# kotaro-kinoshita/yomitoku

Measured on AMD Instinct MI355X. Metric: pages/sec (DocumentAnalyzer @1600x1200, lite model set), higher is better.
Workload: dtype f32 held as two scaled fp16 planes per operand on the MFMA pipe: 3 x v_mfma_f32_32x32x16_f16 per product tile (products to 2^-21, below the fp32 accumulation's own rounding), fp32 accumulate, fp32 activations in HBM; attention, LayerNorm, the fused greedy step and every grid-starved launch exact fp3

## Files before the change

yomitoku_amd/csrc/ymk_api.cpp:

```cpp
#include "../../include/ymk.h"
#include "ymk_common.h"
#include "ymk_decstep.h"
#include "ymk_det.h"
#include "ymk_entry.h"
#include "ymk_seq.h"

struct ymk_model {
  ymk::Model* impl = nullptr;
  int device = 0;
};

#include <dlfcn.h>
namespace {
struct Roctx {
  int (*push)(const char*) = nullptr;
  int (*pop)() = nullptr;
  Roctx() {
    const char* on = std::getenv("YMK_ROCTX");
    if (on == nullptr || on[0] == '\0' || on[0] == '0') return;
    for (const char* name : {"librocprofiler-sdk-roctx.so", "libroctx64.so"}) {
      if (void* h = dlopen(name, RTLD_NOW | RTLD_GLOBAL)) {
        push = reinterpret_cast<int (*)(const char*)>(dlsym(h, "roctxRangePushA"));
        pop = reinterpret_cast<int (*)()>(dlsym(h, "roctxRangePop"));
        if (push && pop) return;
// ... 26 lines not shown
    return 1;                                       \
  }                                                 \
  catch (...) {                                     \
    ymk::set_error("unknown C++ exception");        \
    return 2;                                       \
  }

extern "C" {

int ymk_version(void) { return 100; }

const char* ymk_last_error(void) { return ymk::last_error().c_str(); }

int ymk_device_count(void) {
  int n = 0;
  if (hipGetDeviceCount(&n) != hipSuccess) return -1;
  return n;
}

ymk_model* ymk_model_create(const char* kind, int device) {
  try {
    YMK_CHECK(kind != nullptr, "kind is null");
    YMK_HIP(hipSetDevice(device));
    std::string k(kind);
    ymk::Model* impl = nullptr;
    if (k == "dbnet") impl = ymk::create_dbnet();
    else if (k == "parseq") impl = ymk::create_parseq();
    else if (k == "rtdetr") impl = ymk::create_rtdetr();
    else throw ymk::Error("unknown model kind: " + k);
    auto* m = new ymk_model();
    m->impl = impl;
    m->device = device;
    return m;
  } catch (const std::exception& e) {
    ymk::set_error(e.what());
    return nullptr;
  }
}

void ymk_model_destroy(ymk_model* m) {
  if (!m) return;
  (void)hipSetDevice(m->device);
  delete m->impl;
  delete m;
}

int ymk_model_set_param(ymk_model* m, const char* key, double value) {
  YMK_API_BEGIN
  YMK_CHECK(m && key, "null argument");
  const std::string k(key);
  if (k == "workspace_reuse") {
    YMK_CHECK(value == 0.0 || value == 1.0 || value == -1.0, "workspace_reuse must be 0 or 1 (-1: follow the process-wide default)");
    YMK_CHECK(!ymk::in_forward(), "workspace_reuse cannot change inside a forward");
  }
  m->impl->params[key] = value;
  if (m->impl->finalized && (k == "conv_split" || k == "conv_split_encoder")) {
    YMK_HIP(hipSetDevice(m->device));
    m->impl->prebuild_split();
  }
  YMK_API_END
}

int ymk_model_set_tensor(ymk_model* m, const char* name, const float* host_data, int ndim, const int64_t* dims) {
  YMK_API_BEGIN
  YMK_CHECK(m && name && host_data && (ndim == 0 || dims), "null argument");
  YMK_CHECK(!m->impl->finalized, "model already finalized");
  m->impl->ws.put(name, host_data, ndim, dims);
  YMK_API_END
}

int ymk_model_finalize(ymk_model* m) {
  YMK_API_BEGIN
  RoctxRange roctx_range("ymk_model_finalize");
  YMK_CHECK(m, "null model");
  YMK_HIP(hipSetDevice(m->device));
  m->impl->finalize();
  m->impl->prebuild_split();
  if (!ymk::debug_hazard_no_finalize_sync()) YMK_HIP(hipDeviceSynchronize());
  YMK_API_END
}

int ymk_model_reserve(ymk_model* m, int n, int h, int w, void* stream) {
  YMK_API_BEGIN
  RoctxRange roctx_range("ymk_model_reserve");
  YMK_CHECK(m && m->impl, "null argument");
  YMK_HIP(hipSetDevice(m->device));
  m->impl->reserve(n, h, w, (hipStream_t)stream);
  YMK_API_END
}

int64_t ymk_model_weight_bytes(const ymk_model* m) { return m ? (int64_t)m->impl->pool.bytes() : -1; }
int64_t ymk_model_workspace_bytes(const ymk_model* m) { return m ? (int64_t)m->impl->arena.capacity() : -1; }

int ymk_dbnet_forward(ymk_model* m, const float* x_dev, int n, int h, int w, float* prob_dev, void* stream) {
  YMK_API_BEGIN
  RoctxRange roctx_range("ymk_dbnet_forward");
  YMK_CHECK(m && x_dev && prob_dev, "null argument");
  YMK_HIP(hipSetDevice(m->device));
  ymk::dbnet_forward(m->impl, x_dev, n, h, w, prob_dev, (hipStream_t)stream);
  YMK_API_END
}

int ymk_parseq_dims(ymk_model* m, int* num_steps, int* num_classes) {
  YMK_API_BEGIN
  YMK_CHECK(m && num_steps && num_classes, "null argument");
  ymk::parseq_dims(m->impl, num_steps, num_classes);
  YMK_API_END
}

int ymk_parseq_forward(ymk_model* m, const float* x_dev, int b, int w, float* logits_dev, int* out_len, int* ar_steps,
                       void* stream) {
  YMK_API_BEGIN
  RoctxRange roctx_range("ymk_parseq_forward");
  YMK_CHECK(m && x_dev && logits_dev && out_len && ar_steps, "null argument");
  YMK_HIP(hipSetDevice(m->device));
  ymk::parseq_forward(m->impl, x_dev, b, w, logits_dev, out_len, ar_steps, (hipStream_t)stream);
  YMK_API_END
}

int ymk_parseq_forward_groups(ymk_model* m, const float* const* x_dev, const int* b, const int* w, int n_groups,
                              float* logits_dev, int* out_len, int* ar_steps, void* stream) {
  YMK_API_BEGIN
  RoctxRange roctx_range("ymk_parseq_forward_groups");
  YMK_CHECK(m && x_dev && b && w && logits_dev && out_len && ar_steps, "null argument");
  YMK_HIP(hipSetDevice(m->device));
  ymk::parseq_forward_groups(m->impl, x_dev, b, w, n_groups, logits_dev, out_len, ar_steps, (hipStream_t)stream);
  YMK_API_END
}

int ymk_parseq_token_stats(const float* logits_dev, int rows, int num_classes, int* ids_dev, float* probs_dev,
                           void* stream) {
  YMK_API_BEGIN
  RoctxRange roctx_range("ymk_parseq_token_stats");
  YMK_CHECK(logits_dev && ids_dev && probs_dev, "null argument");
  ymk::row_maxprob((hipStream_t)stream, logits_dev, rows, num_classes, ids_dev, probs_dev);
  YMK_API_END
}

int ymk_rtdetr_forward(ymk_model* m, const float* x_dev, int b, int h, int w, float* logits_dev, float* boxes_dev,
                       void* stream) {
  YMK_API_BEGIN
  RoctxRange roctx_range("ymk_rtdetr_forward");
  YMK_CHECK(m && x_dev && logits_dev && boxes_dev, "null argument");
  YMK_HIP(hipSetDevice(m->device));
  ymk::rtdetr_forward(m->impl, x_dev, b, h, w, logits_dev, boxes_dev, (hipStream_t)stream);
  YMK_API_END
}

int ymk_debug_option(const char* key, int value) {
  YMK_API_BEGIN
  YMK_CHECK(key != nullptr, "null key");
  const std::string k(key);
  YMK_CHECK(ymk::conv_debug_option(k, value) || ymk::parseq_debug_option(k, value) || ymk::decstep_debug_option(k, value) ||
                ymk::conv_split_debug_option(k, value) || ymk::runtime_debug_option(k, value),
            "unknown debug option: " + k);
  YMK_API_END
}

int ymk_stat(const char* key, int64_t* value) {
  YMK_API_BEGIN
  YMK_CHECK(key != nullptr && value != nullptr, "null argument");
  long long v = 0;
  YMK_CHECK(ymk::conv_split_stat(std::string(key), &v) || ymk::runtime_stat(std::string(key), &v) || ymk::parseq_stat(std::string(key), &v), std::string("unknown counter: ") + key);
  *value = v;
  YMK_API_END
}

int ymk_amax_check_counters(int64_t* out4) {
  YMK_API_BEGIN
  YMK_CHECK(out4 != nullptr, "null argument");
  long long v[4];
  ymk::amax_check_counters(v);
  for (int i = 0; i < 4; ++i) out4[i] = v[i];
  YMK_API_END
}

int ymk_prof_begin(void) {
  YMK_API_BEGIN
  ymk::prof_begin();
  YMK_API_END
}

int ymk_prof_end(double* conv_ms, double* conv_flop, int64_t* conv_launches) {
  YMK_API_BEGIN
  YMK_CHECK(conv_ms && conv_flop && conv_launches, "null argument");
  ymk::prof_end(conv_ms, conv_flop, conv_launches);
  YMK_API_END
}

int ymk_prof_bytes(double* conv_bytes) {
  YMK_API_BEGIN
  YMK_CHECK(conv_bytes, "null argument");
  *conv_bytes = ymk::prof_bytes();
  YMK_API_END
}

int ymk_prof_launch_table(double* ms, double* flop, double* bytes, double* mfma_products, int64_t capacity, int64_t* count) {
  YMK_API_BEGIN
  YMK_CHECK(count != nullptr && capacity >= 0 && (capacity == 0 || (ms && flop && bytes && mfma_products)), "null argument");
  *count = ymk::prof_launch_table(ms, flop, bytes, mfma_products, capacity);
  YMK_API_END
}

int ymk_op_plan_workspace(int64_t n, const int64_t* sizes, const int64_t* release_pos, int64_t* offsets_out, int64_t* peak_out,
                          int64_t* live_bound_out) {
  YMK_API_BEGIN
  YMK_CHECK(n >= 0 && (n == 0 || (sizes && offsets_out)), "plan_workspace: bad argument");
  std::vector<size_t> sz((size_t)n), off((size_t)n);
  for (int64_t k = 0; k < n; ++k) {
    YMK_CHECK(sizes[k] >= 0, "plan_workspace: negative size");
    sz[(size_t)k] = (size_t)sizes[k];
  }
  size_t peak = 0, live = 0;
  ymk::plan_workspace((size_t)n, sz.data(), release_pos, off.data(), &peak, &live);
  for (int64_t k = 0; k < n; ++k) offsets_out[k] = (int64_t)off[(size_t)k];
  if (peak_out) *peak_out = (int64_t)peak;
  if (live_bound_out) *live_bound_out = (int64_t)live;
  YMK_API_END
}

int ymk_op_conv2d(const float* x_dev, int n, int h, int w, int c, const float* w_host_oihw, int cout, int cin, int kh,
                  int kw, const float* scale_host, const float* bias_host, const float* res_dev, int stride, int pad,
                  int dil, int act, int tap4, float* y_dev, void* stream) {
  YMK_API_BEGIN
  using namespace ymk;
  DevicePool pool;
  ConvW cw;
  cw.cout = cout;
  cw.cin = tap4 ? 4 : cin;
  cw.kh = kh;
  cw.kw = kw;
  cw.mode = tap4 ? 1 : 0;
  std::vector<float> panel;
  pack_conv_weight(w_host_oihw, cout, cin, kh, kw, tap4 != 0, panel, cw.kpad, cw.ctiles);
  cw.w = pool.upload(panel);
  if (scale_host) cw.scale = pool.upload(scale_host, cout);
  if (bias_host) cw.bias = pool.upload(bias_host, cout);
  Tensor in{const_cast<float*>(x_dev), n, h, w, c, c};
  const int oh = conv_out_dim(h, kh, stride, pad, dil), ow = conv_out_dim(w, kw, stride, pad, dil);
  Tensor out{y_dev, n, oh, ow, cout, cout};
  Tensor res{const_cast<float*>(res_dev), n, oh, ow, cout, cout};
  ConvArgs a;
  a.stride = stride;
  a.pad = pad;
  a.dil = dil;
  a.act = act;
  a.res = res_dev ? &res : nullptr;
  SplitCtxOwner split_ctx;
  ConvSplitScope scope(-1, split_ctx.get(), 0);
  conv2d((hipStream_t)stream, in, cw, a, out);
  YMK_HIP(hipStreamSynchronize((hipStream_t)stream));
  YMK_API_END
}

int ymk_op_conv1x1_astat(const float* x_dev, int m, int c, const float* w_host_oc, int cout, const float* scale_host,
                         const float* bias_host, const float* res_dev, int act, const float* ln_g_host, const float* ln_b_host, float ln_eps,
                         float* y_dev, int reps, float* kernel_ms, void* stream) {
  YMK_API_BEGIN
  using namespace ymk;
  YMK_CHECK(x_dev && w_host_oc && y_dev && m > 0 && c > 0 && cout > 0, "bad argument");
  YMK_CHECK((ln_g_host == nullptr) == (ln_b_host == nullptr), "LayerNorm: gamma and beta come together");
  hipStream_t s = (hipStream_t)stream;
  DevicePool pool;
  ConvW cw;
  cw.cout = cout;
  cw.cin = c;
  std::vector<float> panel;
  YMK_CHECK(c % 4 == 0, "astat: channels must be a multiple of 4");
  pack_conv_weight(w_host_oc, cout, c, 1, 1, false, panel, cw.kpad, cw.ctiles);
  YMK_CHECK(cw.kpad <= 256, "astat: K <= 256");
  cw.w = pool.upload(panel);
  if (scale_host) cw.scale = pool.upload(scale_host, cout);
  if (bias_host) cw.bias = pool.upload(bias_host, cout);
  unsigned* rec = nullptr;
  const float *g_dev = nullptr, *b_dev = nullptr;
  if (ln_g_host) {
    const std::vector<float> g(ln_g_host, ln_g_host + c), b(ln_b_host, ln_b_host + c);
    g_dev = pool.upload(g);
    b_dev = pool.upload(b);
    rec = make_layernorm_amax_record(pool, g, b);
  } else {
    rec = reinterpret_cast<unsigned*>(pool.alloc(AMAX_REC_WORDS));
    YMK_HIP(hipMemsetAsync(rec, 0, AMAX_REC_WORDS * sizeof(unsigned), s));
    absmax_record(s, x_dev, (size_t)m * c, rec);
  }
  struct Events {
    hipEvent_t e0 = nullptr, e1 = nullptr;
    ~Events() {
      if (e0) (void)hipEventDestroy(e0);
      if (e1) (void)hipEventDestroy(e1);
    }
  } ev;
  YMK_HIP(hipEventCreate(&ev.e0));
  YMK_HIP(hipEventCreate(&ev.e1));
  SplitCtxOwner split_ctx;
  ConvSplitScope scope(SPLIT_F16X2, split_ctx.get(), 0);
  ConvSplitTileScope tile_scope(30);
  for (int r = 0; r < std::max(1, reps); ++r) {
    if (r == std::max(1, reps) - 1) YMK_HIP(hipEventRecord(ev.e0, s));
    if (ln_g_host) {
      YMK_CHECK(gemm_ln_fused(s, x_dev, m, c, c, g_dev, b_dev, ln_eps, cw, act, res_dev, cout, y_dev, cout, rec),
                "astat: this launch cannot carry a fused LayerNorm (C must be 128 or 192)");
    } else {
      YMK_CHECK(gemm_takes_astat(m, c, cw, res_dev != nullptr, cout), "astat: not a launch the A-stationary kernel runs");
      gemm(s, x_dev, m, c, c, cw, act, res_dev, cout, y_dev, cout, nullptr, nullptr, EPI_STORE, rec);
    }
    if (r == std::max(1, reps) - 1) YMK_HIP(hipEventRecord(ev.e1, s));
  }
  YMK_HIP(hipStreamSynchronize(s));
  float ms = 0.f;
  YMK_HIP(hipEventElapsedTime(&ms, ev.e0, ev.e1));
  if (kernel_ms) *kernel_ms = ms;
  YMK_API_END
}

int ymk_op_vit_mlp(const float* x_dev, int m, int d, int f, const float* ln_g_host, const float* ln_b_host, float ln_eps,
// ... 365 lines not shown
```

yomitoku_amd/csrc/ymk_entry.h:

```cpp
#pragma once
#include "ymk_common.h"

namespace ymk {

void dbnet_forward(Model* m, const float* x, int n, int h, int w, float* prob, hipStream_t s);
Model* create_parseq();
void parseq_forward(Model* m, const float* x, int B, int W, float* logits, int* out_len, int* ar_steps, hipStream_t s);
void parseq_forward_groups(Model* m, const float* const* x, const int* b, const int* w, int ng, float* logits, int* out_len,
                           int* ar_steps, hipStream_t s);
void parseq_dims(Model* m, int* num_steps, int* num_classes);
bool parseq_debug_option(const std::string& key, int value);
bool parseq_stat(const std::string& key, long long* value);
Model* create_rtdetr();
void rtdetr_forward(Model* m, const float* x, int B, int H, int W, float* logits, float* boxes, hipStream_t s);

void prof_begin();
void prof_end(double* ms, double* flop, int64_t* launches);
double prof_bytes();
int64_t prof_launch_table(double* ms, double* flop, double* bytes, double* products, int64_t capacity);
bool conv_debug_option(const std::string& key, int value);

bool conv_split_debug_option(const std::string& key, int value);
bool conv_split_stat(const std::string& key, long long* value);
void amax_check_counters(long long* out4);
bool gemm_takes_astat(int M, int K, const ConvW& w, bool with_res, int ld);

}
```

yomitoku_amd/csrc/ymk_seq.hip:

```cpp
#include "ymk_common.h"
#include "ymk_f16_planes.h"
#include "ymk_seq.h"

namespace ymk {


__device__ __forceinline__ float wave_sum(float v) {
#pragma unroll
  for (int o = 32; o > 0; o >>= 1) v += __shfl_xor(v, o, 64);
  return v;
}
__device__ __forceinline__ float wave_max(float v) {
#pragma unroll
  for (int o = 32; o > 0; o >>= 1) v = fmaxf(v, __shfl_xor(v, o, 64));
  return v;
}

__global__ void k_layernorm(const float* __restrict__ x, int ldx, int in_rows_mod, const float* __restrict__ g,
                            const float* __restrict__ b, float eps, float* __restrict__ y, int ldy, int M, int D) {
  const int row = blockIdx.x * (blockDim.x >> 6) + (threadIdx.x >> 6);
  const int lane = threadIdx.x & 63;
  if (row >= M) return;
  const float* xr = x + (size_t)(in_rows_mod > 0 ? row % in_rows_mod : row) * ldx;
  float4 v[4];
  const int nv = D >> 2;
  float s = 0.f;
#pragma unroll
  for (int i = 0; i < 4; ++i) {
    const int c = lane + 64 * i;
    if (c < nv) {
      v[i] = *reinterpret_cast<const float4*>(xr + c * 4);
      s += (v[i].x + v[i].y) + (v[i].z + v[i].w);
    }
  }
  const float mean = wave_sum(s) / (float)D;
  float q = 0.f;
#pragma unroll
  for (int i = 0; i < 4; ++i) {
    const int c = lane + 64 * i;
    if (c < nv) {
      const float a = v[i].x - mean, bb = v[i].y - mean, cc = v[i].z - mean, d = v[i].w - mean;
      q += (a * a + bb * bb) + (cc * cc + d * d);
    }
  }
  const float rstd = 1.f / sqrtf(wave_sum(q) / (float)D + eps);
#pragma unroll
  for (int i = 0; i < 4; ++i) {
    const int c = lane + 64 * i;
    if (c < nv) {
      const float4 gg = *reinterpret_cast<const float4*>(g + c * 4);
      const float4 be = *reinterpret_cast<const float4*>(b + c * 4);
      float4 o;
      o.x = (v[i].x - mean) * rstd * gg.x + be.x;
      o.y = (v[i].y - mean) * rstd * gg.y + be.y;
      o.z = (v[i].z - mean) * rstd * gg.z + be.z;
      o.w = (v[i].w - mean) * rstd * gg.w + be.w;
      *reinterpret_cast<float4*>(y + (size_t)row * ldy + c * 4) = o;
    }
  }
}
void layernorm(hipStream_t s, const float* x, int ldx, int in_rows_mod, const float* g, const float* b, float eps,
               float* y, int ldy, int M, int D) {
  YMK_CHECK(D % 4 == 0 && D <= 1024, "layernorm: D must be a multiple of 4, <= 1024");
  if (M == 0) return;
  hipLaunchKernelGGL(k_layernorm, dim3((M + 3) / 4), dim3(256), 0, s, x, ldx, in_rows_mod, g, b, eps, y, ldy, M, D);
  YMK_HIP(hipGetLastError());
}

__global__ void k_add_pos(float* __restrict__ x, const float* __restrict__ pos, int gh, int gw, int full_gw, int D4,
                          size_t total) {
  for (size_t i = (size_t)blockIdx.x * blockDim.x + threadIdx.x; i < total; i += (size_t)gridDim.x * blockDim.x) {
    const int c4 = (int)(i % D4);
    const size_t tok = i / D4;
    const int cc = (int)(tok % gw);
    const int rr = (int)((tok / gw) % gh);
    float4 v = reinterpret_cast<float4*>(x)[i];
    const float4 p = reinterpret_cast<const float4*>(pos)[(size_t)(rr * full_gw + cc) * D4 + c4];
    v.x += p.x; v.y += p.y; v.z += p.z; v.w += p.w;
    reinterpret_cast<float4*>(x)[i] = v;
  }
}
void add_pos_embed(hipStream_t s, float* x, const float* pos, int B, int gh, int gw, int full_gw, int D) {
  const size_t total = (size_t)B * gh * gw * (D / 4);
  size_t g = (total + 255) / 256;
  if (g > 4096) g = 4096;
  hipLaunchKernelGGL(k_add_pos, dim3((int)g), dim3(256), 0, s, x, pos, gh, gw, full_gw, D / 4, total);
  YMK_HIP(hipGetLastError());
}

struct AttnP {
  const float *q, *k, *v;
  float* o;
  int ldq, ldk, ldv, ldo;
  long bsq, bsk, bsv, bso;
  int Lq, Lk, H;
  float scale;
  const int *qoff, *qlen, *koff, *klen;
  const unsigned *amax_q, *amax_k, *amax_v;
};

template <int HD, int HDR = HD>
__global__ __launch_bounds__(256, 1) void k_flash_attn(AttnP p) {
  constexpr int KT = 64;
  constexpr int LDH = HD + 4;
  constexpr int NKC = HDR / 8;
  constexpr int NDC = HD / 32;
  constexpr int LPT = (KT * HDR / 4) / 256;
  static_assert(HD % 32 == 0 && HDR % 8 == 0 && HDR <= HD && (KT * HDR / 4) % 256 == 0, "head dim");
  __shared__ __attribute__((aligned(16))) float lds[2 * 2 * KT * LDH];

  const int t = threadIdx.x, wv = t >> 6, lane = t & 63, li = lane & 31, lh = lane >> 5;
  const int b = blockIdx.z, h = blockIdx.y;
  const int q0 = blockIdx.x * 128 + wv * 32;
  const float* qb = p.q + (size_t)b * p.bsq + h * HDR;
  const float* kb = p.k + (size_t)b * p.bsk + h * HDR;
  const float* vb = p.v + (size_t)b * p.bsv + h * HDR;
  float* ob = p.o + (size_t)b * p.bso + h * HDR;
  int Lq = p.Lq, Lk = p.Lk;
  if (p.koff) {
    const size_t r = (size_t)p.koff[b];
    kb = p.k + r * p.ldk + h * HDR;
    vb = p.v + r * p.ldv + h * HDR;
    Lk = p.klen[b];
  }
  if (p.qoff) {
    const size_t r = (size_t)p.qoff[b];
    qb = p.q + r * p.ldq + h * HDR;
    ob = p.o + r * p.ldo + h * HDR;
    Lq = p.qlen[b];
  }
  if ((int)blockIdx.x * 128 >= Lq) return;

  f32x4 qf[NKC];
  {
    const int qi = min(q0 + li, Lq - 1);
    const float* qr = qb + (size_t)qi * p.ldq;
#pragma unroll
    for (int kc = 0; kc < NKC; ++kc) {
      qf[kc] = *reinterpret_cast<const f32x4*>(qr + kc * 8 + lh * 4);
      qf[kc] *= p.scale;
    }
  }

  f32x16 oacc[NDC];
#pragma unroll
  for (int dc = 0; dc < NDC; ++dc)
#pragma unroll
    for (int r = 0; r < 16; ++r) oacc[dc][r] = 0.f;
  float m_run = -INFINITY, l_run = 0.f;

  f32x4 rk[LPT], rv[LPT];
  auto load_kv = [&](int k0) {
#pragma unroll
    for (int i = 0; i < LPT; ++i) {
      const int idx = t + 256 * i;
      const int row = idx / (HDR / 4), c4 = idx - row * (HDR / 4);
      const int key = min(k0 + row, Lk - 1);
      rk[i] = *reinterpret_cast<const f32x4*>(kb + (size_t)key * p.ldk + c4 * 4);
      rv[i] = *reinterpret_cast<const f32x4*>(vb + (size_t)key * p.ldv + c4 * 4);
    }
  };
  auto store_kv = [&](int buf) {
    float* Ks = lds + buf * (2 * KT * LDH);
    float* Vs = Ks + KT * LDH;
#pragma unroll
    for (int i = 0; i < LPT; ++i) {
      const int idx = t + 256 * i;
      const int row = idx / (HDR / 4), c4 = idx - row * (HDR / 4);
      *reinterpret_cast<f32x4*>(Ks + row * LDH + c4 * 4) = rk[i];
      *reinterpret_cast<f32x4*>(Vs + row * LDH + c4 * 4) = rv[i];
    }
  };

  const int ntiles = (Lk + KT - 1) / KT;
  load_kv(0);
  store_kv(0);
  __syncthreads();
  for (int tt = 0; tt < ntiles; ++tt) {
    const int buf = tt & 1;
    if (tt + 1 < ntiles) load_kv((tt + 1) * KT);
    const float* Ks = lds + buf * (2 * KT * LDH);
    const float* Vs = Ks + KT * LDH;
#pragma unroll
    for (int sub = 0; sub < (q0 < Lq ? KT / 32 : 0); ++sub) {
      const int kbase = tt * KT + sub * 32;
      if (kbase >= Lk) break;
      f32x16 sacc;
#pragma unroll
      for (int r = 0; r < 16; ++r) sacc[r] = 0.f;
      const float* kr = Ks + (sub * 32 + li) * LDH + lh * 4;
#pragma unroll
      for (int kc = 0; kc < NKC; ++kc) {
        const f32x4 kf = *reinterpret_cast<const f32x4*>(kr + kc * 8);
        sacc = __builtin_amdgcn_mfma_f32_32x32x2f32(kf.x, qf[kc].x, sacc, 0, 0, 0);
        sacc = __builtin_amdgcn_mfma_f32_32x32x2f32(kf.y, qf[kc].y, sacc, 0, 0, 0);
        sacc = __builtin_amdgcn_mfma_f32_32x32x2f32(kf.z, qf[kc].z, sacc, 0, 0, 0);
        sacc = __builtin_amdgcn_mfma_f32_32x32x2f32(kf.w, qf[kc].w, sacc, 0, 0, 0);
      }
      float mt = -INFINITY;
#pragma unroll
      for (int r = 0; r < 16; ++r) {
        const int key = kbase + (r & 3) + 8 * (r >> 2) + 4 * lh;
        if (key >= Lk) sacc[r] = -INFINITY;
        mt = fmaxf(mt, sacc[r]);
      }
      mt = fmaxf(mt, __shfl_xor(mt, 32, 64));
      const float m_new = fmaxf(m_run, mt);
      const float alpha = __expf(m_run - m_new);
      float ps = 0.f;
#pragma unroll
      for (int r = 0; r < 16; ++r) {
        sacc[r] = __expf(sacc[r] - m_new);
        ps += sacc[r];
      }
      ps += __shfl_xor(ps, 32, 64);
      l_run = l_run * alpha + ps;
      m_run = m_new;
#pragma unroll
      for (int dc = 0; dc < NDC; ++dc) {
#pragma unroll
        for (int r = 0; r < 16; ++r) oacc[dc][r] *= alpha;
        const float* vr = Vs + (sub * 32 + 4 * lh) * LDH + dc * 32 + li;
#pragma unroll
        for (int r = 0; r < 16; ++r) {
          const float vf = vr[((r & 3) + 8 * (r >> 2)) * LDH];
          oacc[dc] = __builtin_amdgcn_mfma_f32_32x32x2f32(vf, sacc[r], oacc[dc], 0, 0, 0);
        }
      }
    }
    if (tt + 1 < ntiles) store_kv(buf ^ 1);
    __syncthreads();
  }
  const int qi = q0 + li;
  if (qi < Lq) {
    const float inv = 1.f / l_run;
    float* orow = ob + (size_t)qi * p.ldo;
#pragma unroll
    for (int dc = 0; dc < NDC; ++dc)
#pragma unroll
      for (int g = 0; g < 4; ++g) {
        f32x4 w;
        w.x = oacc[dc][4 * g + 0] * inv;
        w.y = oacc[dc][4 * g + 1] * inv;
        w.z = oacc[dc][4 * g + 2] * inv;
        w.w = oacc[dc][4 * g + 3] * inv;
        if (dc * 32 + 8 * g + 4 * lh < HDR) *reinterpret_cast<f32x4*>(orow + dc * 32 + 8 * g + 4 * lh) = w;
      }
  }
}

template <int HD, int HDR = HD>
__global__ __launch_bounds__(256, (HD <= 32 ? 3 : (HD <= 64 ? 2 : 1))) void k_flash_attn_f16(AttnP p) {
  constexpr int KT = 64;
  constexpr int LDH = HD + 4;
  constexpr int NKS = HDR / 16;
  constexpr int NDC = HD / 32;
  constexpr int LPT = (KT * HDR / 4) / 256;
  static_assert(HD % 32 == 0 && HDR % 16 == 0 && HDR <= HD && (KT * HDR / 4) % 256 == 0, "head dim");
  __shared__ __attribute__((aligned(16))) float lds[2 * 2 * KT * LDH];

  const int t = threadIdx.x, wv = t >> 6, lane = t & 63, li = lane & 31, lh = lane >> 5;
  const int b = blockIdx.z, h = blockIdx.y;
  const int q0 = blockIdx.x * 128 + wv * 32;
  const float* qb = p.q + (size_t)b * p.bsq + h * HDR;
  const float* kb = p.k + (size_t)b * p.bsk + h * HDR;
  const float* vb = p.v + (size_t)b * p.bsv + h * HDR;
  float* ob = p.o + (size_t)b * p.bso + h * HDR;
  int Lq = p.Lq, Lk = p.Lk;
  if (p.koff) {
    const size_t r = (size_t)p.koff[b];
    kb = p.k + r * p.ldk + h * HDR;
    vb = p.v + r * p.ldv + h * HDR;
    Lk = p.klen[b];
  }
  if (p.qoff) {
    const size_t r = (size_t)p.qoff[b];
    qb = p.q + r * p.ldq + h * HDR;
    ob = p.o + r * p.ldo + h * HDR;
    Lq = p.qlen[b];
  }
  if ((int)blockIdx.x * 128 >= Lq) return;

  const float2 cq = f16_plane_scales((unsigned)__builtin_amdgcn_readfirstlane((int)amax_read(p.amax_q, t)));
  const float2 ck = f16_plane_scales((unsigned)__builtin_amdgcn_readfirstlane((int)amax_read(p.amax_k, t)));
  const float2 cv = f16_plane_scales((unsigned)__builtin_amdgcn_readfirstlane((int)amax_read(p.amax_v, t)));
  const float s_q = cq.x, s_k = ck.x, s_v = cv.x;
  const float s_unscale = cq.y * ck.y;
  const float o_unscale = cv.y * (1.f / 16384.f);

  f16x8 qh[NKS], ql[NKS];
  {
    const int qi = min(q0 + li, Lq - 1);
    const float* qr = qb + (size_t)qi * p.ldq;
#pragma unroll
    for (int ks = 0; ks < NKS; ++ks) {
      const f32x4 a = *reinterpret_cast<const f32x4*>(qr + ks * 16 + lh * 8);
      const f32x4 c = *reinterpret_cast<const f32x4*>(qr + ks * 16 + lh * 8 + 4);
      const float x[8] = {a.x * p.scale, a.y * p.scale, a.z * p.scale, a.w * p.scale, c.x * p.scale, c.y * p.scale, c.z * p.scale, c.w * p.scale};
      f16_split8(x, s_q, qh[ks], ql[ks]);
    }
  }

  f32x16 oacc[NDC];
#pragma unroll
  for (int dc = 0; dc < NDC; ++dc)
#pragma unroll
    for (int r = 0; r < 16; ++r) oacc[dc][r] = 0.f;
  float m_run = -INFINITY, l_run = 0.f;

  f32x4 rk[LPT], rv[LPT];
  auto load_kv = [&](int k0) {
#pragma unroll
    for (int i = 0; i < LPT; ++i) {
      const int idx = t + 256 * i;
      const int row = idx / (HDR / 4), c4 = idx - row * (HDR / 4);
      const int key = min(k0 + row, Lk - 1);
      rk[i] = *reinterpret_cast<const f32x4*>(kb + (size_t)key * p.ldk + c4 * 4);
      rv[i] = *reinterpret_cast<const f32x4*>(vb + (size_t)key * p.ldv + c4 * 4);
    }
  };
  auto store_kv = [&](int buf) {
    float* Ks = lds + buf * (2 * KT * LDH);
    float* Vs = Ks + KT * LDH;
#pragma unroll
    for (int i = 0; i < LPT; ++i) {
      const int idx = t + 256 * i;
      const int row = idx / (HDR / 4), c4 = idx - row * (HDR / 4);
      *reinterpret_cast<f32x4*>(Ks + row * LDH + c4 * 4) = rk[i];
      *reinterpret_cast<f32x4*>(Vs + row * LDH + c4 * 4) = rv[i];
    }
  };

  const int ntiles = (Lk + KT - 1) / KT;
  load_kv(0);
  store_kv(0);
  __syncthreads();
  for (int tt = 0; tt < ntiles; ++tt) {
    const int buf = tt & 1;
    if (tt + 1 < ntiles) load_kv((tt + 1) * KT);
    const float* Ks = lds + buf * (2 * KT * LDH);
    const float* Vs = Ks + KT * LDH;
#pragma unroll
    for (int sub = 0; sub < (q0 < Lq ? KT / 32 : 0); ++sub) {
      const int kbase = tt * KT + sub * 32;
      if (kbase >= Lk) break;
      f32x16 sacc;
#pragma unroll
      for (int r = 0; r < 16; ++r) sacc[r] = 0.f;
      const float* kr = Ks + (sub * 32 + li) * LDH + lh * 8;
#pragma unroll
      for (int ks = 0; ks < NKS; ++ks) {
        const f32x4 a = *reinterpret_cast<const f32x4*>(kr + ks * 16);
        const f32x4 c = *reinterpret_cast<const f32x4*>(kr + ks * 16 + 4);
        const float x[8] = {a.x, a.y, a.z, a.w, c.x, c.y, c.z, c.w};
        f16x8 kh, kl;
        f16_split8(x, s_k, kh, kl);
        sacc = __builtin_amdgcn_mfma_f32_32x32x16_f16(kl, qh[ks], sacc, 0, 0, 0);
        sacc = __builtin_amdgcn_mfma_f32_32x32x16_f16(kh, ql[ks], sacc, 0, 0, 0);
        sacc = __builtin_amdgcn_mfma_f32_32x32x16_f16(kh, qh[ks], sacc, 0, 0, 0);
      }
      float mt = -INFINITY;
#pragma unroll
      for (int r = 0; r < 16; ++r) {
        const int key = kbase + (r & 3) + 8 * (r >> 2) + 4 * lh;
        sacc[r] = key >= Lk ? -INFINITY : sacc[r] * s_unscale;
        mt = fmaxf(mt, sacc[r]);
      }
      mt = fmaxf(mt, __shfl_xor(mt, 32, 64));
      const float m_new = fmaxf(m_run, mt);
      const float alpha = __expf(m_run - m_new);
      float ps = 0.f;
#pragma unroll
      for (int r = 0; r < 16; ++r) {
        sacc[r] = __expf(sacc[r] - m_new);
        ps += sacc[r];
      }
      ps += __shfl_xor(ps, 32, 64);
      l_run = l_run * alpha + ps;
      m_run = m_new;
      f16x8 ph[2], pl[2];
#pragma unroll
      for (int j = 0; j < 2; ++j) {
        const float x[8] = {sacc[8 * j], sacc[8 * j + 1], sacc[8 * j + 2], sacc[8 * j + 3], sacc[8 * j + 4], sacc[8 * j + 5], sacc[8 * j + 6], sacc[8 * j + 7]};
        f16_split8(x, 16384.f, ph[j], pl[j]);
      }
#pragma unroll
      for (int dc = 0; dc < NDC; ++dc) {
#pragma unroll
        for (int r = 0; r < 16; ++r) oacc[dc][r] *= alpha;
        const float* vr = Vs + (sub * 32 + 4 * lh) * LDH + dc * 32 + li;
#pragma unroll
        for (int j = 0; j < 2; ++j) {
          float x[8];
#pragma unroll
          for (int e = 0; e < 8; ++e) {
            const int r = 8 * j + e;
            x[e] = vr[((r & 3) + 8 * (r >> 2)) * LDH];
          }
          f16x8 vh, vl;
          f16_split8(x, s_v, vh, vl);
          oacc[dc] = __builtin_amdgcn_mfma_f32_32x32x16_f16(vl, ph[j], oacc[dc], 0, 0, 0);
          oacc[dc] = __builtin_amdgcn_mfma_f32_32x32x16_f16(vh, pl[j], oacc[dc], 0, 0, 0);
          oacc[dc] = __builtin_amdgcn_mfma_f32_32x32x16_f16(vh, ph[j], oacc[dc], 0, 0, 0);
        }
      }
    }
    if (tt + 1 < ntiles) store_kv(buf ^ 1);
    __syncthreads();
  }
  const int qi = q0 + li;
  if (qi < Lq) {
    const float inv = o_unscale / l_run;
    float* orow = ob + (size_t)qi * p.ldo;
#pragma unroll
    for (int dc = 0; dc < NDC; ++dc)
#pragma unroll
      for (int g = 0; g < 4; ++g) {
        f32x4 w;
        w.x = oacc[dc][4 * g + 0] * inv;
        w.y = oacc[dc][4 * g + 1] * inv;
        w.z = oacc[dc][4 * g + 2] * inv;
        w.w = oacc[dc][4 * g + 3] * inv;
        if (dc * 32 + 8 * g + 4 * lh < HDR) *reinterpret_cast<f32x4*>(orow + dc * 32 + 8 * g + 4 * lh) = w;
      }
  }
}

void flash_attention(hipStream_t s, const float* q, const float* k, const float* v, float* o, int B, int H, int Lq, int Lk,
                     int hd, int ldq, int ldk, int ldv, int ldo, long bsq, long bsk, long bsv, long bso, float scale,
                     const SeqTab* tab, const unsigned* amax_q, const unsigned* amax_k, const unsigned* amax_v) {
  if (B == 0 || Lq == 0) return;
  YMK_CHECK(Lk > 0, "attention: no keys");
  YMK_CHECK(ldq % 4 == 0 && ldk % 4 == 0 && ldv % 4 == 0 && ldo % 4 == 0, "attention: strides must be multiples of 4");
  AttnP p{q, k, v, o, ldq, ldk, ldv, ldo, bsq, bsk, bsv, bso, Lq, Lk, H, scale, nullptr, nullptr, nullptr, nullptr, amax_q, amax_k, amax_v};
  if (tab) {
    p.qoff = tab->qoff;
    p.qlen = tab->qlen;
    p.koff = tab->koff;
    p.klen = tab->klen;
    YMK_CHECK((p.qoff == nullptr) == (p.qlen == nullptr) && (p.koff == nullptr) == (p.klen == nullptr), "attention: offset and length tables come in pairs");
  }
  dim3 grid((Lq + 127) / 128, H, B);
  const bool f16 = amax_q && amax_k && amax_v && scale <= 1.f && scale > 0.f && conv_effective_split() == SPLIT_F16X2 && ldq % 4 == 0;
  if (f16 && (hd == 32 || hd == 64 || hd == 96 || hd == 48)) {
    if (hd == 32) hipLaunchKernelGGL(k_flash_attn_f16<32>, grid, dim3(256), 0, s, p);
    else if (hd == 64) hipLaunchKernelGGL(k_flash_attn_f16<64>, grid, dim3(256), 0, s, p);
    else if (hd == 96) hipLaunchKernelGGL(k_flash_attn_f16<96>, grid, dim3(256), 0, s, p);
    else hipLaunchKernelGGL((k_flash_attn_f16<64, 48>), grid, dim3(256), 0, s, p);
    YMK_HIP(hipGetLastError());
    return;
  }
  if (hd == 32) hipLaunchKernelGGL(k_flash_attn<32>, grid, dim3(256), 0, s, p);
  else if (hd == 64) hipLaunchKernelGGL(k_flash_attn<64>, grid, dim3(256), 0, s, p);
  else if (hd == 96) hipLaunchKernelGGL(k_flash_attn<96>, grid, dim3(256), 0, s, p);
  else if (hd == 48) hipLaunchKernelGGL((k_flash_attn<64, 48>), grid, dim3(256), 0, s, p);
  else {
    YMK_CHECK(Lk <= 1024 && hd <= 128, "attention: head dim " + std::to_string(hd) + " is only supported for <= 1024 keys per sample");
    small_attention(s, q, k, v, o, B, H, Lq, Lk, hd, ldq, ldk, ldv, ldo, bsq, bsk, bsv, bso, scale, nullptr, 0, nullptr, 0, tab);
    return;
  }
  YMK_HIP(hipGetLastError());
}

struct SmallAttnP {
  const float *q, *k, *v;
  float* o;
  int ldq, ldk, ldv, ldo;
  long bsq, bsk, bsv, bso;
  int Lq, Lk, H, hd;
  float scale;
  const unsigned char* mask_qk;
  int ld_mask;
  const unsigned char* kpm;
  int ld_kpm;
  const int *koff, *klen;
  const int *qoff, *qlen;
  int vec4;
};
__global__ __launch_bounds__(64) void k_small_attn(SmallAttnP p) {
  __shared__ float prob[1024];
  __shared__ float qs[128];
  const int lane = threadIdx.x;
  const int qi = blockIdx.x, h = blockIdx.y, b = blockIdx.z;
  if (p.qoff && qi >= p.qlen[b]) return;
  const size_t qrow0 = p.qoff ? (size_t)p.qoff[b] : 0;
  const float* qr = (p.qoff ? p.q + qrow0 * p.ldq : p.q + (size_t)b * p.bsq) + (size_t)qi * p.ldq + h * p.hd;
  for (int d = lane; d < p.hd; d += 64) qs[d] = qr[d] * p.scale;
  __syncthreads();
  const float* kb = p.k + (size_t)b * p.bsk + h * p.hd;
  const float* vb = p.v + (size_t)b * p.bsv + h * p.hd;
  int Lk = p.Lk;
  if (p.koff) {
    kb = p.k + (size_t)p.koff[b] * p.ldk + h * p.hd;
    vb = p.v + (size_t)p.koff[b] * p.ldv + h * p.hd;
    Lk = p.klen[b];
  }
  float mx = -INFINITY;
  for (int k = lane; k < Lk; k += 64) {
    bool blocked = false;
    if (p.mask_qk) blocked = p.mask_qk[(size_t)qi * p.ld_mask + k] != 0;
    if (p.kpm) blocked = blocked || p.kpm[(size_t)b * p.ld_kpm + k] != 0;
    float sc = -INFINITY;
    if (!blocked) {
      const float* kr = kb + (size_t)k * p.ldk;
      float a = 0.f;
      if (p.vec4) {
        for (int d = 0; d < p.hd; d += 4) {
          const float4 kk = *reinterpret_cast<const float4*>(kr + d);
          a += qs[d] * kk.x + qs[d + 1] * kk.y + qs[d + 2] * kk.z + qs[d + 3] * kk.w;
        }
      } else {
        for (int d = 0; d < p.hd; ++d) a += qs[d] * kr[d];
      }
      sc = a;
    }
    prob[k] = sc;
    mx = fmaxf(mx, sc);
  }
  mx = wave_max(mx);
  float sum = 0.f;
  for (int k = lane; k < Lk; k += 64) {
    const float e = __expf(prob[k] - mx);
    prob[k] = e;
    sum += e;
  }
  sum = wave_sum(sum);
  __syncthreads();
  const float inv = 1.f / sum;
  float* orow = (p.qoff ? p.o + qrow0 * p.ldo : p.o + (size_t)b * p.bso) + (size_t)qi * p.ldo + h * p.hd;
  for (int d = lane; d < p.hd; d += 64) {
    float a = 0.f;
    for (int k = 0; k < Lk; ++k) a += prob[k] * vb[(size_t)k * p.ldv + d];
    orow[d] = a * inv;
  }
}
void small_attention(hipStream_t s, const float* q, const float* k, const float* v, float* o, int B, int H, int Lq, int Lk,
                     int hd, int ldq, int ldk, int ldv, int ldo, long bsq, long bsk, long bsv, long bso, float scale,
                     const unsigned char* mask_qk, int ld_mask, const unsigned char* kpm, int ld_kpm, const SeqTab* tab) {
  if (B == 0 || Lq == 0) return;
  YMK_CHECK(Lk > 0 && Lk <= 1024 && hd <= 128, "small attention: Lk <= 1024, hd <= 128");
  const int vec4 = hd % 4 == 0 && ldk % 4 == 0 && bsk % 4 == 0 && ((uintptr_t)k & 15) == 0;
  SmallAttnP p{q, k, v, o, ldq, ldk, ldv, ldo, bsq, bsk, bsv, bso, Lq, Lk, H, hd, scale, mask_qk, ld_mask, kpm, ld_kpm,
               tab ? tab->koff : nullptr, tab ? tab->klen : nullptr, tab ? tab->qoff : nullptr, tab ? tab->qlen : nullptr, vec4};
  YMK_CHECK(!tab || (!mask_qk && !kpm), "small attention: ragged batches come without masks");
  hipLaunchKernelGGL(k_small_attn, dim3(Lq, H, B), dim3(64), 0, s, p);
  YMK_HIP(hipGetLastError());
}

__global__ void k_ctx_embed_ln(const int* __restrict__ tok, int ld_tok, int pos0, int npos, const float* __restrict__ emb,
                               const float* __restrict__ posq, const float* __restrict__ g, const float* __restrict__ be,
                               float eps, float sqrt_d, float* __restrict__ out, int out_rows, int D, int B) {
  const int w = blockIdx.x * (blockDim.x >> 6) + (threadIdx.x >> 6);
  const int lane = threadIdx.x & 63;
  if (w >= B * npos) return;
  const int b = w / npos, pos = pos0 + (w - b * npos);
  const int token = tok[(size_t)b * ld_tok + pos];
  const float* er = emb + (size_t)token * D;
  const float* pr = pos > 0 ? posq + (size_t)(pos - 1) * D : nullptr;
  float v[16];
  float s = 0.f;
  const int per = (D + 63) / 64;
  for (int i = 0; i < per; ++i) {
    const int c = lane + 64 * i;
    float x = 0.f;
    if (c < D) {
      x = sqrt_d * er[c];
      if (pr) x = pr[c] + x;
      s += x;
    }
    v[i] = x;
  }
  const float mean = wave_sum(s) / (float)D;
  float q = 0.f;
  for (int i = 0; i < per; ++i) {
    const int c = lane + 64 * i;
    if (c < D) q += (v[i] - mean) * (v[i] - mean);
  }
  const float rstd = 1.f / sqrtf(wave_sum(q) / (float)D + eps);
  float* orow = out + ((size_t)b * out_rows + pos) * D;
  for (int i = 0; i < per; ++i) {
    const int c = lane + 64 * i;
    if (c < D) orow[c] = (v[i] - mean) * rstd * g[c] + be[c];
  }
}
void ctx_embed_ln(hipStream_t s, const int* tok, int ld_tok, int pos0, int npos, const float* emb, const float* posq,
                  const float* g, const float* be, float eps, float* out, int out_rows, int D, int B) {
  YMK_CHECK(D <= 1024, "ctx_embed: D <= 1024");
  const int waves = B * npos;
  if (waves == 0) return;
  hipLaunchKernelGGL(k_ctx_embed_ln, dim3((waves + 3) / 4), dim3(256), 0, s, tok, ld_tok, pos0, npos, emb, posq, g, be, eps,
                     sqrtf((float)D), out, out_rows, D, B);
  YMK_HIP(hipGetLastError());
}

constexpr int ROW_RV = 32;
template <bool WITH_SUM>
__device__ __forceinline__ void row_reduce_256(const float* __restrict__ row, int C, float* sv, int* si, float& mx, int& am,
                                               float& sum) {
  const int t = threadIdx.x;
  float best = -INFINITY;
  int bi = t < C ? t : 0x7fffffff;
// ... 296 lines not shown
```

Before: 125.9.

## Store attention K/V tiles as pre-split swizzled fp16 planes in LDS

The f16 flash-attention kernel now splits each K/V tile into hi/lo fp16 planes once, when it is staged into LDS. It uses swizzled layouts (V transposed) so the MFMA operands load as single 16-byte vectors. Previously every wave re-split the fp32 values on every subtile and gathered V with strided scalar reads. It also skips key masking for full tiles and skips the accumulator rescale when no lane's max changed. The cost is more complex scattered 2-byte stores for V, with a debug option to fall back to the old path.

```diff
diff --git a/yomitoku_amd/csrc/ymk_api.cpp b/yomitoku_amd/csrc/ymk_api.cpp
--- a/yomitoku_amd/csrc/ymk_api.cpp
+++ b/yomitoku_amd/csrc/ymk_api.cpp
@@ -202,7 +202,7 @@
   YMK_CHECK(key != nullptr, "null key");
   const std::string k(key);
   YMK_CHECK(ymk::conv_debug_option(k, value) || ymk::parseq_debug_option(k, value) || ymk::decstep_debug_option(k, value) ||
-                ymk::conv_split_debug_option(k, value) || ymk::runtime_debug_option(k, value),
+                ymk::conv_split_debug_option(k, value) || ymk::runtime_debug_option(k, value) || ymk::seq_debug_option(k, value),
             "unknown debug option: " + k);
   YMK_API_END
 }
@@ -211,7 +211,7 @@
   YMK_API_BEGIN
   YMK_CHECK(key != nullptr && value != nullptr, "null argument");
   long long v = 0;
-  YMK_CHECK(ymk::conv_split_stat(std::string(key), &v) || ymk::runtime_stat(std::string(key), &v) || ymk::parseq_stat(std::string(key), &v), std::string("unknown counter: ") + key);
+  YMK_CHECK(ymk::conv_split_stat(std::string(key), &v) || ymk::runtime_stat(std::string(key), &v) || ymk::parseq_stat(std::string(key), &v) || ymk::seq_stat(std::string(key), &v), std::string("unknown counter: ") + key);
   *value = v;
   YMK_API_END
 }
diff --git a/yomitoku_amd/csrc/ymk_entry.h b/yomitoku_amd/csrc/ymk_entry.h
--- a/yomitoku_amd/csrc/ymk_entry.h
+++ b/yomitoku_amd/csrc/ymk_entry.h
@@ -25,4 +25,7 @@
 void amax_check_counters(long long* out4);
 bool gemm_takes_astat(int M, int K, const ConvW& w, bool with_res, int ld);
 
+bool seq_debug_option(const std::string& key, int value);
+bool seq_stat(const std::string& key, long long* value);
+
 }
diff --git a/yomitoku_amd/csrc/ymk_seq.hip b/yomitoku_amd/csrc/ymk_seq.hip
--- a/yomitoku_amd/csrc/ymk_seq.hip
+++ b/yomitoku_amd/csrc/ymk_seq.hip
@@ -1,6 +1,9 @@
 #include "ymk_common.h"
+#include "ymk_entry.h"
 #include "ymk_f16_planes.h"
 #include "ymk_seq.h"
+
+#include <atomic>
 
 namespace ymk {
 
@@ -249,7 +252,13 @@
   }
 }
 
-template <int HD, int HDR = HD>
+__device__ __forceinline__ constexpr int attn_k_swz(int slots_per_row, int row) {
+  return slots_per_row == 8 ? (row >> 1) & 7 : (slots_per_row == 6 ? (row >> 3) & 1 : (row >> 2) & 3);
+}
+__device__ __forceinline__ constexpr int attn_v_slot(int kk) { return (kk >> 5) * 4 + ((kk >> 4) & 1) * 2 + ((kk >> 2) & 1); }
+__device__ __forceinline__ constexpr int attn_v_elem(int kk) { return (kk & 3) + 4 * ((kk >> 3) & 1); }
+
+template <int HD, int HDR = HD, bool CUT = true>
 __global__ __launch_bounds__(256, (HD <= 32 ? 3 : (HD <= 64 ? 2 : 1))) void k_flash_attn_f16(AttnP p) {
   constexpr int KT = 64;
   constexpr int LDH = HD + 4;
@@ -257,7 +266,15 @@
   constexpr int NDC = HD / 32;
   constexpr int LPT = (KT * HDR / 4) / 256;
   static_assert(HD % 32 == 0 && HDR % 16 == 0 && HDR <= HD && (KT * HDR / 4) % 256 == 0, "head dim");
-  __shared__ __attribute__((aligned(16))) float lds[2 * 2 * KT * LDH];
+  constexpr int KSR = HDR / 8;
+  constexpr int KROW = 2 * HDR;
+  constexpr int KPL = KT * KROW;
+  constexpr int VROW = 2 * KT;
+  constexpr int VPL = HD * VROW;
+  constexpr int BUFB = CUT ? 2 * KPL + 2 * VPL : 2 * KT * LDH * 4;
+  static_assert(2 * KPL + 2 * VPL <= 2 * KT * LDH * 4, "the planes fit where the fp32 rows did");
+  __shared__ __attribute__((aligned(16))) char lds_raw[2 * BUFB];
+  float* const lds = reinterpret_cast<float*>(lds_raw);
 
   const int t = threadIdx.x, wv = t >> 6, lane = t & 63, li = lane & 31, lh = lane >> 5;
   const int b = blockIdx.z, h = blockIdx.y;
@@ -320,14 +337,41 @@
     }
   };
   auto store_kv = [&](int buf) {
-    float* Ks = lds + buf * (2 * KT * LDH);
-    float* Vs = Ks + KT * LDH;
-#pragma unroll
-    for (int i = 0; i < LPT; ++i) {
-      const int idx = t + 256 * i;
-      const int row = idx / (HDR / 4), c4 = idx - row * (HDR / 4);
-      *reinterpret_cast<f32x4*>(Ks + row * LDH + c4 * 4) = rk[i];
-      *reinterpret_cast<f32x4*>(Vs + row * LDH + c4 * 4) = rv[i];
+    if constexpr (CUT) {
+      char* Kb = lds_raw + buf * BUFB;
+      char* Vb = Kb + 2 * KPL;
+#pragma unroll
+      for (int i = 0; i < LPT; ++i) {
+        const int idx = t + 256 * i;
+        const int row = idx / (HDR / 4), c4 = idx - row * (HDR / 4);
+        uint2 hi, lo;
+        const f32x4 a = rk[i] * s_k;
+        f16_split4(f32x2{a.x, a.y}, f32x2{a.z, a.w}, hi, lo);
+        char* kp = Kb + row * KROW + (((c4 >> 1) ^ attn_k_swz(KSR, row)) << 4) + (c4 & 1) * 8;
+        *reinterpret_cast<uint2*>(kp) = hi;
+        *reinterpret_cast<uint2*>(kp + KPL) = lo;
+        const f32x4 c = rv[i] * s_v;
+        f16_split4(f32x2{c.x, c.y}, f32x2{c.z, c.w}, hi, lo);
+        const int vs = attn_v_slot(row), ve = attn_v_elem(row) * 2;
+        const unsigned hw[2] = {hi.x, hi.y}, lw[2] = {lo.x, lo.y};
+#pragma unroll
+        for (int j = 0; j < 4; ++j) {
+          const int d = c4 * 4 + j;
+          char* vp = Vb + d * VROW + ((vs ^ ((d >> 1) & 7)) << 4) + ve;
+          *reinterpret_cast<unsigned short*>(vp) = (unsigned short)(hw[j >> 1] >> (16 * (j & 1)));
+          *reinterpret_cast<unsigned short*>(vp + VPL) = (unsigned short)(lw[j >> 1] >> (16 * (j & 1)));
+        }
+      }
+    } else {
+      float* Ks = lds + buf * (2 * KT * LDH);
+      float* Vs = Ks + KT * LDH;
+#pragma unroll
+      for (int i = 0; i < LPT; ++i) {
+        const int idx = t + 256 * i;
+        const int row = idx / (HDR / 4), c4 = idx - row * (HDR / 4);
+        *reinterpret_cast<f32x4*>(Ks + row * LDH + c4 * 4) = rk[i];
+        *reinterpret_cast<f32x4*>(Vs + row * LDH + c4 * 4) = rv[i];
+      }
     }
   };
 
@@ -340,6 +384,8 @@
     if (tt + 1 < ntiles) load_kv((tt + 1) * KT);
     const float* Ks = lds + buf * (2 * KT * LDH);
     const float* Vs = Ks + KT * LDH;
+    const char* Kb = lds_raw + buf * BUFB;
+    const char* Vb = Kb + 2 * KPL;
 #pragma unroll
     for (int sub = 0; sub < (q0 < Lq ? KT / 32 : 0); ++sub) {
       const int kbase = tt * KT + sub * 32;
@@ -347,24 +393,46 @@
       f32x16 sacc;
 #pragma unroll
       for (int r = 0; r < 16; ++r) sacc[r] = 0.f;
-      const float* kr = Ks + (sub * 32 + li) * LDH + lh * 8;
-#pragma unroll
-      for (int ks = 0; ks < NKS; ++ks) {
-        const f32x4 a = *reinterpret_cast<const f32x4*>(kr + ks * 16);
-        const f32x4 c = *reinterpret_cast<const f32x4*>(kr + ks * 16 + 4);
-        const float x[8] = {a.x, a.y, a.z, a.w, c.x, c.y, c.z, c.w};
-        f16x8 kh, kl;
-        f16_split8(x, s_k, kh, kl);
-        sacc = __builtin_amdgcn_mfma_f32_32x32x16_f16(kl, qh[ks], sacc, 0, 0, 0);
-        sacc = __builtin_amdgcn_mfma_f32_32x32x16_f16(kh, ql[ks], sacc, 0, 0, 0);
-        sacc = __builtin_amdgcn_mfma_f32_32x32x16_f16(kh, qh[ks], sacc, 0, 0, 0);
+      if constexpr (CUT) {
+        const char* kr = Kb + (sub * 32 + li) * KROW;
+        const int ksw = attn_k_swz(KSR, sub * 32 + li);
+#pragma unroll
+        for (int ks = 0; ks < NKS; ++ks) {
+          const char* ka = kr + (((2 * ks + lh) ^ ksw) << 4);
+          const f16x8 kh = *reinterpret_cast<const f16x8*>(ka);
+          const f16x8 kl = *reinterpret_cast<const f16x8*>(ka + KPL);
+          sacc = __builtin_amdgcn_mfma_f32_32x32x16_f16(kl, qh[ks], sacc, 0, 0, 0);
+          sacc = __builtin_amdgcn_mfma_f32_32x32x16_f16(kh, ql[ks], sacc, 0, 0, 0);
+          sacc = __builtin_amdgcn_mfma_f32_32x32x16_f16(kh, qh[ks], sacc, 0, 0, 0);
+        }
+      } else {
+        const float* kr = Ks + (sub * 32 + li) * LDH + lh * 8;
+#pragma unroll
+        for (int ks = 0; ks < NKS; ++ks) {
+          const f32x4 a = *reinterpret_cast<const f32x4*>(kr + ks * 16);
+          const f32x4 c = *reinterpret_cast<const f32x4*>(kr + ks * 16 + 4);
+          const float x[8] = {a.x, a.y, a.z, a.w, c.x, c.y, c.z, c.w};
+          f16x8 kh, kl;
+          f16_split8(x, s_k, kh, kl);
+          sacc = __builtin_amdgcn_mfma_f32_32x32x16_f16(kl, qh[ks], sacc, 0, 0, 0);
+          sacc = __builtin_amdgcn_mfma_f32_32x32x16_f16(kh, ql[ks], sacc, 0, 0, 0);
+          sacc = __builtin_amdgcn_mfma_f32_32x32x16_f16(kh, qh[ks], sacc, 0, 0, 0);
+        }
       }
       float mt = -INFINITY;
-#pragma unroll
-      for (int r = 0; r < 16; ++r) {
-        const int key = kbase + (r & 3) + 8 * (r >> 2) + 4 * lh;
-        sacc[r] = key >= Lk ? -INFINITY : sacc[r] * s_unscale;
-        mt = fmaxf(mt, sacc[r]);
+      if (CUT && kbase + 32 <= Lk) {
+#pragma unroll
+        for (int r = 0; r < 16; ++r) {
+          sacc[r] *= s_unscale;
+          mt = fmaxf(mt, sacc[r]);
+        }
+      } else {
+#pragma unroll
+        for (int r = 0; r < 16; ++r) {
+          const int key = kbase + (r & 3) + 8 * (r >> 2) + 4 * lh;
+          sacc[r] = key >= Lk ? -INFINITY : sacc[r] * s_unscale;
+          mt = fmaxf(mt, sacc[r]);
+        }
       }
       mt = fmaxf(mt, __shfl_xor(mt, 32, 64));
       const float m_new = fmaxf(m_run, mt);
@@ -384,24 +452,42 @@
         const float x[8] = {sacc[8 * j], sacc[8 * j + 1], sacc[8 * j + 2], sacc[8 * j + 3], sacc[8 * j + 4], sacc[8 * j + 5], sacc[8 * j + 6], sacc[8 * j + 7]};
         f16_split8(x, 16384.f, ph[j], pl[j]);
       }
+      const bool rescale = !CUT || __builtin_amdgcn_ballot_w64(alpha != 1.0f) != 0;
 #pragma unroll
       for (int dc = 0; dc < NDC; ++dc) {
-#pragma unroll
-        for (int r = 0; r < 16; ++r) oacc[dc][r] *= alpha;
-        const float* vr = Vs + (sub * 32 + 4 * lh) * LDH + dc * 32 + li;
-#pragma unroll
-        for (int j = 0; j < 2; ++j) {
-          float x[8];
-#pragma unroll
-          for (int e = 0; e < 8; ++e) {
-            const int r = 8 * j + e;
-            x[e] = vr[((r & 3) + 8 * (r >> 2)) * LDH];
+        if (rescale) {
+#pragma unroll
+          for (int r = 0; r < 16; ++r) oacc[dc][r] *= alpha;
+        }
+        if constexpr (CUT) {
+          const int d = dc * 32 + li;
+          const char* vr = Vb + d * VROW;
+          const int vsw = (d >> 1) & 7;
+#pragma unroll
+          for (int j = 0; j < 2; ++j) {
+            const char* va = vr + (((sub * 4 + j * 2 + lh) ^ vsw) << 4);
+            const f16x8 vh = *reinterpret_cast<const f16x8*>(va);
+            const f16x8 vl = *reinterpret_cast<const f16x8*>(va + VPL);
+            oacc[dc] = __builtin_amdgcn_mfma_f32_32x32x16_f16(vl, ph[j], oacc[dc], 0, 0, 0);
+            oacc[dc] = __builtin_amdgcn_mfma_f32_32x32x16_f16(vh, pl[j], oacc[dc], 0, 0, 0);
+            oacc[dc] = __builtin_amdgcn_mfma_f32_32x32x16_f16(vh, ph[j], oacc[dc], 0, 0, 0);
           }
-          f16x8 vh, vl;
-          f16_split8(x, s_v, vh, vl);
-          oacc[dc] = __builtin_amdgcn_mfma_f32_32x32x16_f16(vl, ph[j], oacc[dc], 0, 0, 0);
-          oacc[dc] = __builtin_amdgcn_mfma_f32_32x32x16_f16(vh, pl[j], oacc[dc], 0, 0, 0);
-          oacc[dc] = __builtin_amdgcn_mfma_f32_32x32x16_f16(vh, ph[j], oacc[dc], 0, 0, 0);
+        } else {
+          const float* vr = Vs + (sub * 32 + 4 * lh) * LDH + dc * 32 + li;
+#pragma unroll
+          for (int j = 0; j < 2; ++j) {
+            float x[8];
+#pragma unroll
+            for (int e = 0; e < 8; ++e) {
+              const int r = 8 * j + e;
+              x[e] = vr[((r & 3) + 8 * (r >> 2)) * LDH];
+            }
+            f16x8 vh, vl;
+            f16_split8(x, s_v, vh, vl);
+            oacc[dc] = __builtin_amdgcn_mfma_f32_32x32x16_f16(vl, ph[j], oacc[dc], 0, 0, 0);
+            oacc[dc] = __builtin_amdgcn_mfma_f32_32x32x16_f16(vh, pl[j], oacc[dc], 0, 0, 0);
+            oacc[dc] = __builtin_amdgcn_mfma_f32_32x32x16_f16(vh, ph[j], oacc[dc], 0, 0, 0);
+          }
         }
       }
     }
@@ -424,6 +510,20 @@
         if (dc * 32 + 8 * g + 4 * lh < HDR) *reinterpret_cast<f32x4*>(orow + dc * 32 + 8 * g + 4 * lh) = w;
       }
   }
+}
+
+static std::atomic<int> g_attn_kv_cut{1};
+static std::atomic<long long> g_n_attn_tile_cut{0}, g_n_attn_wave_cut{0};
+bool seq_debug_option(const std::string& key, int value) {
+  if (key != "attn_kv_cut") return false;
+  g_attn_kv_cut = value;
+  return true;
+}
+bool seq_stat(const std::string& key, long long* value) {
+  if (key == "attn_tile_cut_launches") *value = g_n_attn_tile_cut.load();
+  else if (key == "attn_wave_cut_launches") *value = g_n_attn_wave_cut.load();
+  else return false;
+  return true;
 }
 
 void flash_attention(hipStream_t s, const float* q, const float* k, const float* v, float* o, int B, int H, int Lq, int Lk,
@@ -443,10 +543,19 @@
   dim3 grid((Lq + 127) / 128, H, B);
   const bool f16 = amax_q && amax_k && amax_v && scale <= 1.f && scale > 0.f && conv_effective_split() == SPLIT_F16X2 && ldq % 4 == 0;
   if (f16 && (hd == 32 || hd == 64 || hd == 96 || hd == 48)) {
-    if (hd == 32) hipLaunchKernelGGL(k_flash_attn_f16<32>, grid, dim3(256), 0, s, p);
-    else if (hd == 64) hipLaunchKernelGGL(k_flash_attn_f16<64>, grid, dim3(256), 0, s, p);
-    else if (hd == 96) hipLaunchKernelGGL(k_flash_attn_f16<96>, grid, dim3(256), 0, s, p);
-    else hipLaunchKernelGGL((k_flash_attn_f16<64, 48>), grid, dim3(256), 0, s, p);
+    if (g_attn_kv_cut.load() != 0) {
+      if (hd == 32) hipLaunchKernelGGL((k_flash_attn_f16<32, 32, true>), grid, dim3(256), 0, s, p);
+      else if (hd == 64) hipLaunchKernelGGL((k_flash_attn_f16<64, 64, true>), grid, dim3(256), 0, s, p);
+      else if (hd == 96) hipLaunchKernelGGL((k_flash_attn_f16<96, 96, true>), grid, dim3(256), 0, s, p);
+      else hipLaunchKernelGGL((k_flash_attn_f16<64, 48, true>), grid, dim3(256), 0, s, p);
+      ++g_n_attn_tile_cut;
+    } else {
+      if (hd == 32) hipLaunchKernelGGL((k_flash_attn_f16<32, 32, false>), grid, dim3(256), 0, s, p);
+      else if (hd == 64) hipLaunchKernelGGL((k_flash_attn_f16<64, 64, false>), grid, dim3(256), 0, s, p);
+      else if (hd == 96) hipLaunchKernelGGL((k_flash_attn_f16<96, 96, false>), grid, dim3(256), 0, s, p);
+      else hipLaunchKernelGGL((k_flash_attn_f16<64, 48, false>), grid, dim3(256), 0, s, p);
+      ++g_n_attn_wave_cut;
+    }
     YMK_HIP(hipGetLastError());
     return;
   }
```

After: 123.2. 0.979x the previous value.
